# ed-fish/data-efficient-video-transformers

Measured on AMD Instinct MI355X. Metric: clips/sec fwd+bwd, B=8 T=32 3x224x224 bf16, higher is better.
Workload: dtype bf16; 1 GPU; ViViT metric shape (SURVEY 8 'M'; BASELINE configs[2]/[3] transformer): B=8/GPU, T=32, 3x224x224, patch 16, d=512, ...; global_batch=8, parallelism=dp1

## Files before the change

data-efficient-video-transformers_amd/csrc/attention.hip:

```cpp
#include "common.h"
#include <cstdlib>

namespace {

__device__ __forceinline__ void wave_lds_sync() {
  asm volatile("s_waitcnt lgkmcnt(0)" ::: "memory");
  __builtin_amdgcn_wave_barrier();
}

constexpr float kLog2e = 1.4426950408889634f;
constexpr float kLn2 = 0.6931471805599453f;

struct AttnParams {
  const void *q, *k, *v, *o, *d_o;
  void *out, *dq, *dk, *dv;
  float* lse;
  float* delta;
  int B, H, Lq, Lk, dh;
  int64_t q_sb, q_sh, q_sl, k_sb, k_sh, k_sl, v_sb, v_sh, v_sl, o_sb, o_sh, o_sl;
  float scale;
  int Lkp;
  int Lqp;
  int patch_off;
  uint32_t drop_thr;
// ... 777 lines not shown
  };
  V8 qf[2];
  load_q(wid, qf);
  stage_images<E>(ks, kb, p.k_sl, vs, vb, p.v_sl, p.Lk, NKP * 32);
  __syncthreads();

  const float c2 = p.scale * kLog2e;
  char* patch = p.patch_off >= 0 ? smem + p.patch_off + wid * 2048 : nullptr;
  for (int qt = wid; qt < nqt; qt += W) {
    asm volatile("" ::: "memory");
    f32x4 s[NKP][2];
#pragma unroll
    for (int kp = 0; kp < NKP; ++kp)
#pragma unroll
      for (int tt = 0; tt < 2; ++tt) {
        s[kp][tt] = f32x4{0.f, 0.f, 0.f, 0.f};
#pragma unroll
        for (int kk = 0; kk < 2; ++kk)
          s[kp][tt] = Elem16<E>::mma(img_row_frag<E>(ks, (2 * kp + tt) * 16, kk, g, li), qf[kk], s[kp][tt]);
      }
    load_q(qt + W, qf);
    __builtin_amdgcn_sched_barrier(0);
#pragma unroll
    for (int tt = 0; tt < 2; ++tt)
#pragma unroll
      for (int r = 0; r < 4; ++r)
        if ((2 * (NKP - 1) + tt) * 16 + 4 * g + r >= p.Lk) s[NKP - 1][tt][r] = -INFINITY;
    float mx = vmax2(s[0][0][0], s[0][0][1]);
#pragma unroll
    for (int kp = 0; kp < NKP; ++kp)
#pragma unroll
      for (int tt = 0; tt < 2; ++tt) {
        if (kp == 0 && tt == 0) {
          mx = vmax3(mx, s[0][0][2], s[0][0][3]);
        } else {
          mx = vmax3(mx, s[kp][tt][0], s[kp][tt][1]);
          mx = vmax3(mx, s[kp][tt][2], s[kp][tt][3]);
        }
      }
    mx = rows_allreduce<true>(mx);
    const float mn = mx * c2;
    f32x4 o[4];
#pragma unroll
    for (int dt = 0; dt < 4; ++dt) o[dt] = f32x4{0.f, 0.f, 0.f, 0.f};
    f32x4 ol = f32x4{0.f, 0.f, 0.f, 0.f};
    V8 ones;
#pragma unroll
    for (int j = 0; j < 8; ++j) ones[j] = (E)1.0f;
    const f32x2 c2v = {c2, c2}, mnv = {-mn, -mn};
#pragma unroll
    for (int kp = 0; kp < NKP; ++kp) {
#pragma unroll
      for (int tt = 0; tt < 2; ++tt) {
        const f32x2 a = __builtin_elementwise_fma(f32x2{s[kp][tt][0], s[kp][tt][1]}, c2v, mnv);
        const f32x2 c = __builtin_elementwise_fma(f32x2{s[kp][tt][2], s[kp][tt][3]}, c2v, mnv);
        s[kp][tt][0] = __builtin_amdgcn_exp2f(a[0]);
        s[kp][tt][1] = __builtin_amdgcn_exp2f(a[1]);
        s[kp][tt][2] = __builtin_amdgcn_exp2f(c[0]);
        s[kp][tt][3] = __builtin_amdgcn_exp2f(c[1]);
      }
      const V8 pf = pack_pair<E>(s[kp][0], s[kp][1]);
#pragma unroll
      for (int dt = 0; dt < 4; ++dt)
        o[dt] = Elem16<E>::mma(img_tr_frag<E>(vs, 2 * kp, 2 * kp + 1, dt * 16, g, li), pf, o[dt]);
      ol = Elem16<E>::mma(ones, pf, ol);
    }
    const float l = ol[0];
    const float inv = 1.0f / l;
    const int qi = qt * 16 + li;
    consume(qf[0]);
    consume(qf[1]);
    store_tile<E>(patch, ob, p.o_sl, qt * 16, p.Lq, o, inv, lane);
    if (qi < p.Lq && g == 0) lse[qi] = (mn + __builtin_amdgcn_logf(l)) * kLn2;
  }
}


template <typename E, int NKP>
__global__ __launch_bounds__(1024) void attn_bwd_dq_mfma_kernel(const AttnParams p) {
  extern __shared__ __attribute__((aligned(16))) char smem[];
  using V8 = typename Elem16<E>::v8;
  const int lane = threadIdx.x & 63, wid = threadIdx.x >> 6, W = blockDim.x >> 6;
  const int g = lane >> 4, li = lane & 15;
  const int b = blockIdx.x / p.H, h = blockIdx.x % p.H;
  const E* qb = (const E*)p.q + b * p.q_sb + h * p.q_sh;
  const E* kb = (const E*)p.k + b * p.k_sb + h * p.k_sh;
  const E* vb = (const E*)p.v + b * p.v_sb + h * p.v_sh;
  const E* ob = (const E*)p.o + b * p.o_sb + h * p.o_sh;
  const E* gb = (const E*)p.d_o + b * p.o_sb + h * p.o_sh;
  E* dqb = (E*)p.dq + b * p.q_sb + h * p.q_sh;
  const float* lse = p.lse + ((int64_t)b * p.H + h) * p.Lq;
  float* delta = p.delta + ((int64_t)b * p.H + h) * p.Lq;
  char* ks = smem;
  char* vs = smem + p.Lkp * kRowBytes;
  const int nqt = (p.Lq + 15) >> 4, nkp = NKP ? NKP : p.Lkp >> 5;
  auto load_rows = [&](int qt, V8* qf, V8* gf, V8* of, float& l2) {
    const int qi = qt * 16 + li;
    const int qrow = qi < p.Lq ? qi : p.Lq - 1;
#pragma unroll
    for (int kk = 0; kk < 2; ++kk) {
      qf[kk] = *reinterpret_cast<const V8*>(qb + (int64_t)qrow * p.q_sl + kk * 32 + g * 8);
      gf[kk] = *reinterpret_cast<const V8*>(gb + (int64_t)qrow * p.o_sl + kk * 32 + g * 8);
      of[kk] = *reinterpret_cast<const V8*>(ob + (int64_t)qrow * p.o_sl + kk * 32 + g * 8);
    }
    l2 = lse[qrow] * kLog2e;
  };
  V8 qf[2], gf[2], of[2];
  float l2;
  load_rows(wid, qf, gf, of, l2);
  stage_images<E>(ks, kb, p.k_sl, vs, vb, p.v_sl, p.Lk, p.Lkp);
  __syncthreads();

  const float c2 = p.scale * kLog2e;
  char* patch = p.patch_off >= 0 ? smem + p.patch_off + wid * 2048 : nullptr;
  for (int qt = wid; qt < nqt; qt += W) {
    asm volatile("" ::: "memory");
    float dl = 0.f;
#pragma unroll
    for (int kk = 0; kk < 2; ++kk)
#pragma unroll
      for (int j = 0; j < 8; ++j) dl = fmaf((float)gf[kk][j], (float)of[kk][j], dl);
    dl = rows_allreduce<false>(dl);
    if (g == 0 && qt * 16 + li < p.Lq) delta[qt * 16 + li] = dl;
    V8 qn[2], gn[2];
    float l2n;
    load_rows(qt + W, qn, gn, of, l2n);
    __builtin_amdgcn_sched_barrier(0);
    f32x4 acc[4];
#pragma unroll
    for (int dt = 0; dt < 4; ++dt) acc[dt] = f32x4{0.f, 0.f, 0.f, 0.f};
    const f32x2 c2v = {c2, c2}, l2v = {-l2, -l2}, dlv = {-dl, -dl};
    auto step = [&](int kp, bool last) {
      f32x4 s[2], dp[2];
#pragma unroll
      for (int tt = 0; tt < 2; ++tt) {
        s[tt] = f32x4{0.f, 0.f, 0.f, 0.f};
        dp[tt] = f32x4{0.f, 0.f, 0.f, 0.f};
#pragma unroll
        for (int kk = 0; kk < 2; ++kk) {
          s[tt] = Elem16<E>::mma(img_row_frag<E>(ks, (2 * kp + tt) * 16, kk, g, li), qf[kk], s[tt]);
          dp[tt] = Elem16<E>::mma(img_row_frag<E>(vs, (2 * kp + tt) * 16, kk, g, li), gf[kk], dp[tt]);
        }
      }
#pragma unroll
      for (int tt = 0; tt < 2; ++tt)
#pragma unroll
        for (int r = 0; r < 4; r += 2) {
          const f32x2 x = __builtin_elementwise_fma(f32x2{s[tt][r], s[tt][r + 1]}, c2v, l2v);
          const f32x2 d = f32x2{dp[tt][r], dp[tt][r + 1]} + dlv;
          const f32x2 pr = {__builtin_amdgcn_exp2f(x[0]), __builtin_amdgcn_exp2f(x[1])};
          const f32x2 ds = pr * d;
          s[tt][r] = ds[0];
          s[tt][r + 1] = ds[1];
          if (last && (2 * kp + tt) * 16 + 4 * g + r >= p.Lk) s[tt][r] = 0.f;
          if (last && (2 * kp + tt) * 16 + 4 * g + r + 1 >= p.Lk) s[tt][r + 1] = 0.f;
        }
      const V8 dsf = pack_pair<E>(s[0], s[1]);
#pragma unroll
      for (int dt = 0; dt < 4; ++dt)
        acc[dt] = Elem16<E>::mma(img_tr_frag<E>(ks, 2 * kp, 2 * kp + 1, dt * 16, g, li), dsf, acc[dt]);
    };
    if constexpr (NKP > 0) {
#pragma unroll
      for (int kp = 0; kp < NKP; ++kp) step(kp, kp == NKP - 1);
    } else {
      for (int kp = 0; kp < nkp - 1; ++kp) step(kp, false);
      step(nkp - 1, true);
    }
#pragma unroll
    for (int kk = 0; kk < 2; ++kk) {
      consume(qn[kk]);
      consume(gn[kk]);
      consume(of[kk]);
    }
    consume(l2n);
    store_tile<E>(patch, dqb, p.q_sl, qt * 16, p.Lq, acc, p.scale, lane);
#pragma unroll
    for (int kk = 0; kk < 2; ++kk) {
      qf[kk] = qn[kk];
      gf[kk] = gn[kk];
    }
    l2 = l2n;
  }
}

template <typename E, int NQP>
__global__ __launch_bounds__(1024) void attn_bwd_dkv_mfma_kernel(const AttnParams p) {
  extern __shared__ __attribute__((aligned(16))) char smem[];
  using V8 = typename Elem16<E>::v8;
  const int lane = threadIdx.x & 63, wid = threadIdx.x >> 6, W = blockDim.x >> 6;
  const int g = lane >> 4, li = lane & 15;
  const int b = blockIdx.x / p.H, h = blockIdx.x % p.H;
  const E* qb = (const E*)p.q + b * p.q_sb + h * p.q_sh;
  const E* kb = (const E*)p.k + b * p.k_sb + h * p.k_sh;
  const E* vb = (const E*)p.v + b * p.v_sb + h * p.v_sh;
  const E* gb = (const E*)p.d_o + b * p.o_sb + h * p.o_sh;
  E* dkb = (E*)p.dk + b * p.k_sb + h * p.k_sh;
  E* dvb = (E*)p.dv + b * p.v_sb + h * p.v_sh;
  const float* lse = p.lse + ((int64_t)b * p.H + h) * p.Lq;
  const float* delta = p.delta + ((int64_t)b * p.H + h) * p.Lq;
  char* qs = smem;
  char* gs = smem + p.Lqp * kRowBytes;
  float* l2s = reinterpret_cast<float*>(smem + 2 * p.Lqp * kRowBytes);
  float* dls = l2s + p.Lqp;
  const int nkt = (p.Lk + 15) >> 4, nqp = NQP ? NQP : p.Lqp >> 5;
  auto load_rows = [&](int kt, V8* kf, V8* vf) {
    const int kj = kt * 16 + li;
    const int krow = kj < p.Lk ? kj : p.Lk - 1;
#pragma unroll
    for (int kk = 0; kk < 2; ++kk) {
      kf[kk] = *reinterpret_cast<const V8*>(kb + (int64_t)krow * p.k_sl + kk * 32 + g * 8);
      vf[kk] = *reinterpret_cast<const V8*>(vb + (int64_t)krow * p.v_sl + kk * 32 + g * 8);
    }
  };
  V8 kf[2], vf[2];
  load_rows(wid, kf, vf);
  const int sr = (int)threadIdx.x < p.Lq ? (int)threadIdx.x : p.Lq - 1;
  const float lse0 = lse[sr], dl0 = delta[sr];
  stage_images<E>(qs, qb, p.q_sl, gs, gb, p.o_sl, p.Lq, p.Lqp);
  if ((int)threadIdx.x < p.Lqp) {
    l2s[threadIdx.x] = (int)threadIdx.x < p.Lq ? -lse0 * kLog2e : 0.f;
    dls[threadIdx.x] = (int)threadIdx.x < p.Lq ? -dl0 : 0.f;
  }
  for (int r = threadIdx.x + blockDim.x; r < p.Lqp; r += blockDim.x) {
    l2s[r] = r < p.Lq ? -lse[r] * kLog2e : 0.f;
    dls[r] = r < p.Lq ? -delta[r] : 0.f;
  }
  __syncthreads();

  const float c2 = p.scale * kLog2e;
  char* patch = p.patch_off >= 0 ? smem + p.patch_off + wid * 2048 : nullptr;
  for (int kt = wid; kt < nkt; kt += W) {
    asm volatile("" ::: "memory");
    f32x4 dk[4], dv[4];
#pragma unroll
    for (int dt = 0; dt < 4; ++dt) {
      dk[dt] = f32x4{0.f, 0.f, 0.f, 0.f};
      dv[dt] = f32x4{0.f, 0.f, 0.f, 0.f};
    }
    const f32x2 c2v = {c2, c2};
    auto step = [&](int qp) {
      f32x4 s[2], dp[2];
#pragma unroll
      for (int tt = 0; tt < 2; ++tt) {
        s[tt] = f32x4{0.f, 0.f, 0.f, 0.f};
        dp[tt] = f32x4{0.f, 0.f, 0.f, 0.f};
#pragma unroll
        for (int kk = 0; kk < 2; ++kk) {
          s[tt] = Elem16<E>::mma(img_row_frag<E>(qs, (2 * qp + tt) * 16, kk, g, li), kf[kk], s[tt]);
          dp[tt] = Elem16<E>::mma(img_row_frag<E>(gs, (2 * qp + tt) * 16, kk, g, li), vf[kk], dp[tt]);
        }
      }
#pragma unroll
      for (int tt = 0; tt < 2; ++tt) {
        const int q0 = (2 * qp + tt) * 16 + 4 * g;
        const f32x4 l2 = *reinterpret_cast<const f32x4*>(l2s + q0);
        const f32x4 dl = *reinterpret_cast<const f32x4*>(dls + q0);
#pragma unroll
        for (int r = 0; r < 4; r += 2) {
          const f32x2 x = __builtin_elementwise_fma(f32x2{s[tt][r], s[tt][r + 1]}, c2v, f32x2{l2[r], l2[r + 1]});
          const f32x2 d = f32x2{dp[tt][r], dp[tt][r + 1]} + f32x2{dl[r], dl[r + 1]};
          const f32x2 pr = {__builtin_amdgcn_exp2f(x[0]), __builtin_amdgcn_exp2f(x[1])};
          const f32x2 ds = pr * d;
          s[tt][r] = pr[0];
          s[tt][r + 1] = pr[1];
          dp[tt][r] = ds[0];
          dp[tt][r + 1] = ds[1];
        }
      }
      const V8 pf = pack_pair<E>(s[0], s[1]);
      const V8 dsf = pack_pair<E>(dp[0], dp[1]);
#pragma unroll
      for (int dt = 0; dt < 4; ++dt) {
        dv[dt] = Elem16<E>::mma(img_tr_frag<E>(gs, 2 * qp, 2 * qp + 1, dt * 16, g, li), pf, dv[dt]);
        dk[dt] = Elem16<E>::mma(img_tr_frag<E>(qs, 2 * qp, 2 * qp + 1, dt * 16, g, li), dsf, dk[dt]);
      }
    };
    if constexpr (NQP > 0) {
#pragma unroll
      for (int qp = 0; qp < NQP; ++qp) step(qp);
    } else {
      for (int qp = 0; qp < nqp; ++qp) step(qp);
    }
    if (kt + W < nkt) load_rows(kt + W, kf, vf);
    store_tile<E>(patch, dkb, p.k_sl, kt * 16, p.Lk, dk, p.scale, lane);
    store_tile<E>(patch, dvb, p.v_sl, kt * 16, p.Lk, dv, 1.0f, lane);
  }
}

constexpr int kStripRow = 80;

template <typename E>
__device__ __forceinline__ typename Elem16<E>::v8 strip_tr_frag(const char* strip, int ta, int tb, int col0, int g, int li) {
  const int qq = li >> 2, pp = li & 3;
  typename Elem16<E>::v4 half[2];
#pragma unroll
  for (int hf = 0; hf < 2; ++hf) {
    const int r = 16 * (hf ? tb : ta) + 4 * g + qq;
    half[hf] = Elem16<E>::tr_read(strip + r * kStripRow + col0 * 2 + 8 * pp);
  }
  return __builtin_shufflevector(half[0], half[1], 0, 1, 2, 3, 4, 5, 6, 7);
}

template <typename E, int NCH>
__device__ __forceinline__ void stage_bwd_operands(char* qs, const E* q, int64_t q_sl, char* gs, const E* g, const E* o, int64_t o_sl,
                                                   char* ks, const E* k, int64_t k_sl, int Lq, int Lk, int rows_pad, float* dls) {
  using V8 = typename Elem16<E>::v8;
  const int total = rows_pad * 8, nt = blockDim.x;
  V8 vq[NCH], vg[NCH], vo[NCH], vk[NCH];
#pragma unroll
  for (int u = 0; u < NCH; ++u) {
    const int idx = min((int)threadIdx.x + u * nt, total - 1);
    const int r = idx >> 3, c = idx & 7;
    const int rq = r < Lq ? r : 0, rk = r < Lk ? r : 0;
    vq[u] = *reinterpret_cast<const V8*>(q + (int64_t)rq * q_sl + c * 8);
    vg[u] = *reinterpret_cast<const V8*>(g + (int64_t)rq * o_sl + c * 8);
    vo[u] = *reinterpret_cast<const V8*>(o + (int64_t)rq * o_sl + c * 8);
    vk[u] = *reinterpret_cast<const V8*>(k + (int64_t)rk * k_sl + c * 8);
  }
  __builtin_amdgcn_sched_barrier(0);
  const V8 zero = {0, 0, 0, 0, 0, 0, 0, 0};
#pragma unroll
  for (int u = 0; u < NCH; ++u) {
    const int idx = min((int)threadIdx.x + u * nt, total - 1);
    const int r = idx >> 3, off = img_off(r, idx & 7);
    const bool lq = r < Lq, lk = r < Lk;
    *reinterpret_cast<V8*>(qs + off) = lq ? vq[u] : zero;
    *reinterpret_cast<V8*>(gs + off) = lq ? vg[u] : zero;
    *reinterpret_cast<V8*>(ks + off) = lk ? vk[u] : zero;
    float d = 0.f;
#pragma unroll
    for (int j = 0; j < 8; ++j) d = fmaf((float)vg[u][j], (float)vo[u][j], d);
    d += __shfl_xor(d, 1, 64);
    d += __shfl_xor(d, 2, 64);
    d += __shfl_xor(d, 4, 64);
    if ((idx & 7) == 0) dls[r] = lq ? -d : 0.f;
  }
}

template <typename E, int NP>
__global__ __launch_bounds__(512) void attn_bwd_fused_kernel(const AttnParams p) {
  extern __shared__ __attribute__((aligned(16))) char smem[];
  using V8 = typename Elem16<E>::v8;
  using V4 = typename Elem16<E>::v4;
  constexpr int LP = 32 * NP;
  const int lane = threadIdx.x & 63;
  const int wid = __builtin_amdgcn_readfirstlane(threadIdx.x >> 6);
  const int W = blockDim.x >> 6, WC = W - 1;
  const int g = lane >> 4, li = lane & 15;
  const int b = blockIdx.x / p.H, h = blockIdx.x % p.H;
  const E* qb = (const E*)p.q + b * p.q_sb + h * p.q_sh;
  const E* kb = (const E*)p.k + b * p.k_sb + h * p.k_sh;
  const E* vb = (const E*)p.v + b * p.v_sb + h * p.v_sh;
  const E* ob = (const E*)p.o + b * p.o_sb + h * p.o_sh;
  const E* gb = (const E*)p.d_o + b * p.o_sb + h * p.o_sh;
  E* dqb = (E*)p.dq + b * p.q_sb + h * p.q_sh;
  E* dkb = (E*)p.dk + b * p.k_sb + h * p.k_sh;
  E* dvb = (E*)p.dv + b * p.v_sb + h * p.v_sh;
  const float* lse = p.lse + ((int64_t)b * p.H + h) * p.Lq;
  char* qs = smem;
  char* gs = qs + LP * kRowBytes;
  char* ks = gs + LP * kRowBytes;
  char* strip0 = ks + LP * kRowBytes;
  float* l2s = reinterpret_cast<float*>(strip0 + 2 * LP * kStripRow);
  float* dls = l2s + LP;
  char* patch = reinterpret_cast<char*>(dls + LP) + wid * 2048;

  V8 kf[2][2], vf[2][2];
  if (wid < WC) {
#pragma unroll
    for (int j = 0; j < 2; ++j) {
      const int kj = (2 * wid + j) * 16 + li;
      const int krow = kj < p.Lk ? kj : p.Lk - 1;
#pragma unroll
      for (int kk = 0; kk < 2; ++kk) {
        kf[j][kk] = *reinterpret_cast<const V8*>(kb + (int64_t)krow * p.k_sl + kk * 32 + g * 8);
        vf[j][kk] = *reinterpret_cast<const V8*>(vb + (int64_t)krow * p.v_sl + kk * 32 + g * 8);
      }
    }
  }
  {
    const int r = threadIdx.x;
    const float l = lse[r < p.Lq ? r : 0];
    stage_bwd_operands<E, 4>(qs, qb, p.q_sl, gs, gb, ob, p.o_sl, ks, kb, p.k_sl, p.Lq, p.Lk, LP, dls);
    if (r < LP) l2s[r] = r < p.Lq ? -l * kLog2e : 0.f;
  }
  __syncthreads();
  const float c2 = p.scale * kLog2e;
  if (wid < WC) {
    f32x4 dk[2][4], dv[2][4];
#pragma unroll
    for (int j = 0; j < 2; ++j)
#pragma unroll
      for (int dt = 0; dt < 4; ++dt) {
        dk[j][dt] = f32x4{0.f, 0.f, 0.f, 0.f};
        dv[j][dt] = f32x4{0.f, 0.f, 0.f, 0.f};
      }
    const f32x2 c2v = {c2, c2};
    const bool kvalid[2] = {(2 * wid) * 16 + li < p.Lk, (2 * wid + 1) * 16 + li < p.Lk};
    char* myrow[2] = {strip0 + ((2 * wid) * 16 + li) * kStripRow + g * 8, strip0 + ((2 * wid + 1) * 16 + li) * kStripRow + g * 8};
#pragma unroll
    for (int qp = 0; qp < NP; ++qp) {
      asm volatile("" ::: "memory");
      V8 qfr[2][2], gfr[2][2];
#pragma unroll
      for (int tt = 0; tt < 2; ++tt)
#pragma unroll
        for (int kk = 0; kk < 2; ++kk) {
          qfr[tt][kk] = img_row_frag<E>(qs, (2 * qp + tt) * 16, kk, g, li);
          gfr[tt][kk] = img_row_frag<E>(gs, (2 * qp + tt) * 16, kk, g, li);
        }
      f32x4 l2[2], dl[2];
#pragma unroll
      for (int tt = 0; tt < 2; ++tt) {
        l2[tt] = *reinterpret_cast<const f32x4*>(l2s + (2 * qp + tt) * 16 + 4 * g);
        dl[tt] = *reinterpret_cast<const f32x4*>(dls + (2 * qp + tt) * 16 + 4 * g);
      }
      V8 pf[2], dsf[2];
#pragma unroll
      for (int j = 0; j < 2; ++j) {
        f32x4 s[2], dp[2];
#pragma unroll
        for (int tt = 0; tt < 2; ++tt) {
          s[tt] = f32x4{0.f, 0.f, 0.f, 0.f};
          dp[tt] = f32x4{0.f, 0.f, 0.f, 0.f};
#pragma unroll
          for (int kk = 0; kk < 2; ++kk) {
            s[tt] = Elem16<E>::mma(qfr[tt][kk], kf[j][kk], s[tt]);
            dp[tt] = Elem16<E>::mma(gfr[tt][kk], vf[j][kk], dp[tt]);
          }
        }
#pragma unroll
        for (int tt = 0; tt < 2; ++tt)
#pragma unroll
          for (int r = 0; r < 4; r += 2) {
            const f32x2 x = __builtin_elementwise_fma(f32x2{s[tt][r], s[tt][r + 1]}, c2v, f32x2{l2[tt][r], l2[tt][r + 1]});
            const f32x2 d = f32x2{dp[tt][r], dp[tt][r + 1]} + f32x2{dl[tt][r], dl[tt][r + 1]};
            f32x2 pr = {__builtin_amdgcn_exp2f(x[0]), __builtin_amdgcn_exp2f(x[1])};
            if (!kvalid[j]) pr = f32x2{0.f, 0.f};
            const f32x2 ds = pr * d;
            s[tt][r] = pr[0];
            s[tt][r + 1] = pr[1];
            dp[tt][r] = ds[0];
            dp[tt][r + 1] = ds[1];
          }
        pf[j] = pack_pair<E>(s[0], s[1]);
        dsf[j] = pack_pair<E>(dp[0], dp[1]);
      }
#pragma unroll
      for (int j = 0; j < 2; ++j) {
        char* row = myrow[j] + (qp & 1) * (LP * kStripRow);
        *reinterpret_cast<V4*>(row) = __builtin_shufflevector(dsf[j], dsf[j], 0, 1, 2, 3);
        *reinterpret_cast<V4*>(row + 32) = __builtin_shufflevector(dsf[j], dsf[j], 4, 5, 6, 7);
      }
#pragma unroll
      for (int dt = 0; dt < 4; ++dt) {
        const V8 gt = img_tr_frag<E>(gs, 2 * qp, 2 * qp + 1, dt * 16, g, li);
        const V8 qt = img_tr_frag<E>(qs, 2 * qp, 2 * qp + 1, dt * 16, g, li);
#pragma unroll
        for (int j = 0; j < 2; ++j) {
          dv[j][dt] = Elem16<E>::mma(gt, pf[j], dv[j][dt]);
          dk[j][dt] = Elem16<E>::mma(qt, dsf[j], dk[j][dt]);
        }
      }
      __syncthreads();
    }
#pragma unroll
    for (int j = 0; j < 2; ++j) {
      const int k0 = (2 * wid + j) * 16;
      if (k0 < p.Lk) {
        store_tile<E>(patch, dkb, p.k_sl, k0, p.Lk, dk[j], p.scale, lane);
        store_tile<E>(patch, dvb, p.v_sl, k0, p.Lk, dv[j], 1.0f, lane);
      }
    }
  } else {
    V8 ka[NP][4];
#pragma unroll
    for (int kp = 0; kp < NP; ++kp)
#pragma unroll
      for (int dt = 0; dt < 4; ++dt) ka[kp][dt] = img_tr_frag<E>(ks, 2 * kp, 2 * kp + 1, dt * 16, g, li);
#pragma unroll 1
    for (int qp = 0; qp < NP; ++qp) {
      __syncthreads();
      const char* strip = strip0 + (qp & 1) * (LP * kStripRow);
      V8 bq[NP][2];
#pragma unroll
      for (int kp = 0; kp < NP; ++kp) {
        bq[kp][0] = strip_tr_frag<E>(strip, 2 * kp, 2 * kp + 1, 0, g, li);
        bq[kp][1] = strip_tr_frag<E>(strip, 2 * kp, 2 * kp + 1, 16, g, li);
      }
      f32x4 acc[2][4];
#pragma unroll
      for (int tt = 0; tt < 2; ++tt)
#pragma unroll
        for (int dt = 0; dt < 4; ++dt) acc[tt][dt] = f32x4{0.f, 0.f, 0.f, 0.f};
#pragma unroll
      for (int kp = 0; kp < NP; ++kp)
#pragma unroll
        for (int dt = 0; dt < 4; ++dt) {
          acc[0][dt] = Elem16<E>::mma(ka[kp][dt], bq[kp][0], acc[0][dt]);
          acc[1][dt] = Elem16<E>::mma(ka[kp][dt], bq[kp][1], acc[1][dt]);
        }
#pragma unroll
      for (int tt = 0; tt < 2; ++tt)
        if ((2 * qp + tt) * 16 < p.Lq) store_tile<E>(nullptr, dqb, p.q_sl, (2 * qp + tt) * 16, p.Lq, acc[tt], p.scale, lane);
    }
  }
}

constexpr int kMaxLds = 160 * 1024;

int fill_params(const dvt_attn_desc* d, AttnParams& p, bool bwd, const char* name) {
  DVT_REQUIRE(d, "%s: null descriptor", name);
  DVT_REQUIRE(d->q && d->k && d->v && d->o && d->lse, "%s: null q/k/v/o/lse", name);
  DVT_REQUIRE(d->B >= 0 && d->H > 0 && d->Lq > 0 && d->Lk > 0 && d->dh > 0, "%s: bad sizes", name);
  DVT_REQUIRE(d->B * d->H < (1ll << 31) && d->Lq < (1 << 24) && d->Lk < (1 << 24), "%s: sizes too large", name);
  if (bwd) DVT_REQUIRE(d->d_o && d->dq && d->dk && d->dv, "%s: null gradient pointer", name);
  p.q = d->q; p.k = d->k; p.v = d->v; p.o = d->o; p.out = d->o; p.d_o = d->d_o;
  p.dq = d->dq; p.dk = d->dk; p.dv = d->dv; p.lse = d->lse; p.delta = nullptr;
  p.B = (int)d->B; p.H = (int)d->H; p.Lq = (int)d->Lq; p.Lk = (int)d->Lk; p.dh = (int)d->dh;
  p.q_sb = d->q_sb; p.q_sh = d->q_sh; p.q_sl = d->q_sl;
  p.k_sb = d->k_sb; p.k_sh = d->k_sh; p.k_sl = d->k_sl;
  p.v_sb = d->v_sb; p.v_sh = d->v_sh; p.v_sl = d->v_sl;
  p.o_sb = d->o_sb; p.o_sh = d->o_sh; p.o_sl = d->o_sl;
  p.scale = d->scale;
  DVT_REQUIRE(d->dropout_p >= 0.f && d->dropout_p < 1.f, "%s: dropout_p must be in [0, 1)", name);
  DVT_REQUIRE(d->dropout_p == 0.f || d->rng_state, "%s: dropout needs rng_state", name);
  p.drop_thr = 0u; p.drop_scale = 1.f; p.rng = d->rng_state; p.rng_off = d->rng_offset;
  if (d->dropout_p > 0.f) {
    const double th = (double)d->dropout_p * 4294967296.0;
    p.drop_thr = th >= 4294967295.0 ? 0xFFFFFFFFu : (uint32_t)(th + 0.5);
    if (p.drop_thr == 0u) p.drop_thr = 1u;
    p.drop_scale = 1.0f / (1.0f - d->dropout_p);
  }
  p.Lkp = (p.Lk + 31) & ~31;
  p.Lqp = (p.Lq + 31) & ~31;
  p.patch_off = -1;

  return DVT_OK;
}

bool strides_vec_ok(const dvt_attn_desc* d) {
  const int64_t s[] = {d->q_sb, d->q_sh, d->q_sl, d->k_sb, d->k_sh, d->k_sl,
                       d->v_sb, d->v_sh, d->v_sl, d->o_sb, d->o_sh, d->o_sl};
  for (int64_t x : s)
    if (x % 8) return false;
  return true;
}

bool mfma_fwd_ok(const dvt_attn_desc* d, const AttnParams& p) {
  return d->dropout_p == 0.f && d->scale > 0.f && dvt_is_16bit(d->dtype) && d->dh == DH && strides_vec_ok(d) && dvt_aligned16(d->q) &&
         dvt_aligned16(d->k) && dvt_aligned16(d->v) && dvt_aligned16(d->o) &&
         2 * p.Lkp * kRowBytes <= kMaxLds;
}

bool q1_ok(const dvt_attn_desc* d, const AttnParams& p) {
  return p.Lq == 1 && d->dropout_p == 0.f && dvt_is_16bit(d->dtype) && d->dh == DH && strides_vec_ok(d) &&
         dvt_aligned16(d->q) && dvt_aligned16(d->k) && dvt_aligned16(d->v) && dvt_aligned16(d->o) &&
         (size_t)4 * p.Lkp * sizeof(float) <= (size_t)kMaxLds;
}

bool mfma_bwd_ok(const dvt_attn_desc* d, const AttnParams& p) {
  return mfma_fwd_ok(d, p) && dvt_aligned16(d->d_o) && dvt_aligned16(d->dq) && dvt_aligned16(d->dk) &&
         dvt_aligned16(d->dv) && 2 * p.Lqp * kRowBytes + 2 * p.Lqp * 4 <= kMaxLds;
}

bool fused_bwd_ok(const AttnParams& p) { return p.Lqp == p.Lkp && p.Lkp <= 224; }
size_t fused_bwd_lds(int NP, int waves) {
  const size_t LP = 32 * (size_t)NP;
  return 3 * LP * kRowBytes + 2 * LP * kStripRow + 2 * LP * sizeof(float) + (size_t)waves * 2048;
}

int pick_waves(int tiles, size_t lds_bytes, int cap = 16) {
  int maxw = lds_bytes > 80 * 1024 ? 16 : 8;
  if (maxw > cap) maxw = cap;
  const int rounds = (tiles + maxw - 1) / maxw;
  int w = (tiles + rounds - 1) / rounds;
  return w < 1 ? 1 : w;
}

size_t with_patches(size_t lds, int waves, AttnParams& p) {
  const size_t tot = lds + (size_t)waves * 2048;
  const bool ok = lds <= 80 * 1024 ? 2 * tot <= (size_t)kMaxLds : tot <= (size_t)kMaxLds;
  p.patch_off = ok ? (int)lds : -1;
  return ok ? tot : lds;
}

template <typename K>
int set_lds(K kernel, size_t bytes) {
  if (bytes > 64 * 1024) {
    const hipError_t e = hipFuncSetAttribute((const void*)kernel, hipFuncAttributeMaxDynamicSharedMemorySize, (int)bytes);
    if (e != hipSuccess) return dvt_fail_hip(e, "hipFuncSetAttribute(MaxDynamicSharedMemorySize)");
  }
  return 0;
}

int resolve_fwd(const dvt_attn_desc* d, AttnParams& p, dvt_attn_plan_info& r) {
  r = dvt_attn_plan_info{};
  r.patch = r.patch2 = -1;
  int rc = fill_params(d, p, false, "dvt_attention_fwd");
  if (rc) return rc;
  if (p.B == 0) return DVT_OK;
  if (q1_ok(d, p)) {
    r.family = DVT_ATTN_F_Q1; r.waves = 4; r.lds = (int64_t)4 * p.Lkp * sizeof(float);
    return DVT_OK;
  }
  if (mfma_fwd_ok(d, p)) {
    const size_t lds_img = (size_t)2 * p.Lkp * kRowBytes;
    const int nkp = p.Lkp >> 5;
    r.waves = pick_waves((p.Lq + 15) / 16, lds_img, nkp > 7 && nkp <= 11 ? 12 : 16);
    r.lds = (int64_t)with_patches(lds_img, r.waves, p);
    r.patch = p.patch_off >= 0;
    r.family = nkp <= 11 ? DVT_ATTN_F_RES : DVT_ATTN_F_ONLINE;
    r.count = nkp <= 11 ? nkp : 0;
    return DVT_OK;
  }
  const int nt_s = p.Lq * p.dh >= 4096 ? 512 : 256;
  const size_t lds_s = ((size_t)(p.Lq + 2 * p.Lk) * small_dhp(p.dh) +
                        (size_t)small_parts(p.Lq, p.Lk, nt_s) * p.Lq * small_lp(p.Lk)) * sizeof(float);
  if (d->dtype != DVT_F32 && d->dtype != DVT_BF16 && d->dtype != DVT_F16)
    DVT_UNSUPPORTED("dvt_attention_fwd: dtype %d not supported", d->dtype);
  if (p.Lq <= kSmallL && p.Lk <= kSmallL && p.dh <= kSmallDh && lds_s <= (size_t)kMaxLds) {
    r.family = DVT_ATTN_F_SMALL; r.waves = nt_s / 64; r.lds = (int64_t)lds_s;
    return DVT_OK;
  }
  const size_t lds = (size_t)4 * (p.dh + p.Lk) * sizeof(float);
  if (lds > (size_t)kMaxLds) DVT_UNSUPPORTED("dvt_attention_fwd: Lk = %d, dh = %d exceed the LDS budget", p.Lk, p.dh);
  r.family = DVT_ATTN_F_GENERIC; r.waves = 4; r.lds = (int64_t)lds;
  return DVT_OK;
}

int resolve_bwd(const dvt_attn_desc* d, AttnParams& p, AttnParams& pq, AttnParams& pkv, dvt_attn_plan_info& r) {
  r = dvt_attn_plan_info{};
  r.patch = r.patch2 = -1;
  int rc = fill_params(d, p, true, "dvt_attention_bwd");
  if (rc) return rc;
  pq = pkv = p;
  if (p.B == 0) return DVT_OK;
  if (q1_ok(d, p) && dvt_aligned16(d->d_o) && dvt_aligned16(d->dq) && dvt_aligned16(d->dk) && dvt_aligned16(d->dv)) {
    r.family = DVT_ATTN_B_Q1; r.waves = 4;
    return DVT_OK;
  }
  if (mfma_bwd_ok(d, p) && fused_bwd_ok(p) && !d->bwd_two_pass) {
    const int NP = p.Lkp >> 5;
    r.family = DVT_ATTN_B_FUSED; r.count = NP;
    r.waves = NP + 1;
    r.lds = (int64_t)fused_bwd_lds(NP, r.waves);
    return DVT_OK;
  }
  if (mfma_bwd_ok(d, p)) {
    const size_t img_q = (size_t)2 * p.Lkp * kRowBytes;
    const size_t img_kv = (size_t)2 * p.Lqp * kRowBytes + (size_t)2 * p.Lqp * sizeof(float);
    r.family = DVT_ATTN_B_PAIR; r.workspace = 1;
    r.count = (p.Lkp >> 5) <= 11 ? p.Lkp >> 5 : 0;
    r.count2 = (p.Lqp >> 5) <= 11 ? p.Lqp >> 5 : 0;
    r.waves = pick_waves((p.Lq + 15) / 16, img_q);
    r.waves2 = pick_waves((p.Lk + 15) / 16, img_kv);
    r.lds = (int64_t)with_patches(img_q, r.waves, pq);
    r.lds2 = (int64_t)with_patches(img_kv, r.waves2, pkv);
    r.patch = pq.patch_off >= 0; r.patch2 = pkv.patch_off >= 0;
    return DVT_OK;
  }
  if (d->dtype != DVT_F32 && d->dtype != DVT_BF16 && d->dtype != DVT_F16)
    DVT_UNSUPPORTED("dvt_attention_bwd: dtype %d not supported", d->dtype);
  const int nt_s = p.Lq * p.dh >= 4096 ? 512 : 256;
  const size_t lds_s = ((size_t)2 * (p.Lq + p.Lk) * small_dhp(p.dh) +
                        (size_t)2 * small_parts(p.Lq, p.Lk, nt_s) * p.Lq * small_lp(p.Lk) +
                        (size_t)2 * p.Lk * small_lp(p.Lq)) * sizeof(float);
  if (p.Lq <= kSmallL && p.Lk <= kSmallL && p.dh <= kSmallDh && lds_s <= (size_t)kMaxLds) {
    r.family = DVT_ATTN_B_SMALL; r.waves = nt_s / 64; r.lds = (int64_t)lds_s;
    return DVT_OK;
  }
  const size_t lds_q = (size_t)4 * (2 * p.dh + p.Lk) * sizeof(float);
  const size_t lds_kv = (size_t)4 * (2 * p.dh + 2 * p.Lq) * sizeof(float);
  if (lds_q > (size_t)kMaxLds || lds_kv > (size_t)kMaxLds)
    DVT_UNSUPPORTED("dvt_attention_bwd: Lq = %d, Lk = %d, dh = %d exceed the LDS budget", p.Lq, p.Lk, p.dh);
  r.family = DVT_ATTN_B_GENERIC; r.workspace = 1; r.waves = r.waves2 = 4;
  r.lds = (int64_t)lds_q; r.lds2 = (int64_t)lds_kv;
  return DVT_OK;
}

}

extern "C" {

size_t dvt_attention_bwd_workspace_bytes(const dvt_attn_desc* d) {
  if (!d) return 0;
  return (size_t)d->B * (size_t)d->H * (size_t)d->Lq * sizeof(float);
}

int dvt_attention_plan(const dvt_attn_desc* d, int bwd, dvt_attn_plan_info* info) {
  DVT_REQUIRE(info, "dvt_attention_plan: null info");
  AttnParams p, pq, pkv;
  return bwd ? resolve_bwd(d, p, pq, pkv, *info) : resolve_fwd(d, p, *info);
}

int dvt_attention_fwd(const dvt_attn_desc* d, dvt_stream_t stream) {
  AttnParams p;
  dvt_attn_plan_info r;
  int rc = resolve_fwd(d, p, r);
  if (rc) return rc;
  if (p.B == 0) return DVT_OK;
  hipStream_t st = (hipStream_t)stream;
  const size_t lds = (size_t)r.lds;
  if (r.family == DVT_ATTN_F_Q1) {
    const dim3 grid((unsigned)dvt_cdiv((int64_t)p.B * p.H, 4)), block(256);
    DVT_DISPATCH_16BIT(d->dtype, E, {
      if (int rc_ = set_lds(attn_fwd_q1_kernel<E>, lds)) return rc_;
      hipLaunchKernelGGL((attn_fwd_q1_kernel<E>), grid, block, lds, st, p);
    });
    DVT_LAUNCH_CHECK("dvt_attention_fwd(q1)");
    return DVT_OK;
  }
  if (r.family == DVT_ATTN_F_RES || r.family == DVT_ATTN_F_ONLINE) {
    const dim3 grid((unsigned)(p.B * p.H)), block(64 * r.waves);
#define DVT_ATTN_FWD_RES(NKP)                                                               \
  case NKP:                                                                                 \
    if (int rc_ = set_lds(attn_fwd_mfma_res_kernel<E, NKP>, lds)) return rc_;                                         \
    hipLaunchKernelGGL((attn_fwd_mfma_res_kernel<E, NKP>), grid, block, lds, st, p);        \
    break
    DVT_DISPATCH_16BIT(d->dtype, E, {
      switch (r.count) {
        DVT_ATTN_FWD_RES(1); DVT_ATTN_FWD_RES(2); DVT_ATTN_FWD_RES(3); DVT_ATTN_FWD_RES(4);
        DVT_ATTN_FWD_RES(5); DVT_ATTN_FWD_RES(6); DVT_ATTN_FWD_RES(7); DVT_ATTN_FWD_RES(8);
        DVT_ATTN_FWD_RES(9); DVT_ATTN_FWD_RES(10); DVT_ATTN_FWD_RES(11);
        default:
          if (int rc_ = set_lds(attn_fwd_mfma_kernel<E>, lds)) return rc_;
          hipLaunchKernelGGL((attn_fwd_mfma_kernel<E>), grid, block, lds, st, p);
      }
    });
#undef DVT_ATTN_FWD_RES
    DVT_LAUNCH_CHECK("dvt_attention_fwd(mfma)");
    return DVT_OK;
  }
  if (r.family == DVT_ATTN_F_SMALL) {
    const dim3 grid((unsigned)(p.B * p.H)), block(64 * r.waves);
#define DVT_ATTN_SMALL_FWD(T)                                                   \
  do {                                                                          \
    if (int rc_ = set_lds(attn_small_fwd_kernel<T>, lds)) return rc_;                                   \
    hipLaunchKernelGGL((attn_small_fwd_kernel<T>), grid, block, lds, st, p);  \
  } while (0)
    if (d->dtype == DVT_F32) DVT_ATTN_SMALL_FWD(float);
    else if (d->dtype == DVT_BF16) DVT_ATTN_SMALL_FWD(bf16);
    else DVT_ATTN_SMALL_FWD(f16);
#undef DVT_ATTN_SMALL_FWD
    DVT_LAUNCH_CHECK("dvt_attention_fwd(short)");
    return DVT_OK;
  }
  const int64_t rows = (int64_t)p.B * p.H * p.Lq;
  const dim3 grid((unsigned)dvt_cdiv(rows, 4)), block(256);
  if (d->dtype == DVT_F32) {
    if (int rc_ = set_lds(attn_fwd_generic_kernel<float>, lds)) return rc_;
    hipLaunchKernelGGL((attn_fwd_generic_kernel<float>), grid, block, lds, st, p);
  } else if (d->dtype == DVT_BF16) {
    if (int rc_ = set_lds(attn_fwd_generic_kernel<bf16>, lds)) return rc_;
    hipLaunchKernelGGL((attn_fwd_generic_kernel<bf16>), grid, block, lds, st, p);
  } else {
    if (int rc_ = set_lds(attn_fwd_generic_kernel<f16>, lds)) return rc_;
    hipLaunchKernelGGL((attn_fwd_generic_kernel<f16>), grid, block, lds, st, p);
  }
  DVT_LAUNCH_CHECK("dvt_attention_fwd(generic)");
  return DVT_OK;
}

int dvt_attention_bwd(const dvt_attn_desc* d, dvt_stream_t stream) {
  AttnParams p, pq, pkv;
  dvt_attn_plan_info r;
  int rc = resolve_bwd(d, p, pq, pkv, r);
  if (rc) return rc;
  if (p.B == 0) return DVT_OK;
  hipStream_t st = (hipStream_t)stream;
  if (r.family == DVT_ATTN_B_Q1) {
    const dim3 grid((unsigned)dvt_cdiv((int64_t)p.B * p.H, 4)), block(256);
    DVT_DISPATCH_16BIT(d->dtype, E, hipLaunchKernelGGL((attn_bwd_q1_kernel<E>), grid, block, 0, st, p));
    DVT_LAUNCH_CHECK("dvt_attention_bwd(q1)");
    return DVT_OK;
  }
  if (r.family == DVT_ATTN_B_FUSED) {
    const size_t lds = (size_t)r.lds;
    const dim3 grid((unsigned)(p.B * p.H)), block(64 * r.waves);
#define DVT_ATTN_BWD_FUSED(N)                                                               \
  case N:                                                                                   \
    if (int rc_ = set_lds(attn_bwd_fused_kernel<E, N>, lds)) return rc_;                                              \
    hipLaunchKernelGGL((attn_bwd_fused_kernel<E, N>), grid, block, lds, st, p);             \
    break
    DVT_DISPATCH_16BIT(d->dtype, E, {
      switch (r.count) {
        DVT_ATTN_BWD_FUSED(1); DVT_ATTN_BWD_FUSED(2); DVT_ATTN_BWD_FUSED(3); DVT_ATTN_BWD_FUSED(4);
        DVT_ATTN_BWD_FUSED(5); DVT_ATTN_BWD_FUSED(6); DVT_ATTN_BWD_FUSED(7);
      }
    });
#undef DVT_ATTN_BWD_FUSED
    DVT_LAUNCH_CHECK("dvt_attention_bwd(fused)");
    return DVT_OK;
  }
  if (r.family == DVT_ATTN_B_PAIR) {
    DVT_REQUIRE(d->workspace, "dvt_attention_bwd: workspace (dvt_attention_bwd_workspace_bytes) required");
    pq.delta = pkv.delta = (float*)d->workspace;
    const dim3 grid((unsigned)(p.B * p.H));
    const dim3 block_q(64 * r.waves), block_kv(64 * r.waves2);
    const size_t lds_q = (size_t)r.lds, lds_kv = (size_t)r.lds2;
#define DVT_ATTN_BWD_DQ(NKP)                                                                \
  case NKP:                                                                                 \
    if (int rc_ = set_lds(attn_bwd_dq_mfma_kernel<E, NKP>, lds_q)) return rc_;                                        \
    hipLaunchKernelGGL((attn_bwd_dq_mfma_kernel<E, NKP>), grid, block_q, lds_q, st, pq);     \
    break
#define DVT_ATTN_BWD_DKV(NQP)                                                               \
  case NQP:                                                                                 \
    if (int rc_ = set_lds(attn_bwd_dkv_mfma_kernel<E, NQP>, lds_kv)) return rc_;                                      \
    hipLaunchKernelGGL((attn_bwd_dkv_mfma_kernel<E, NQP>), grid, block_kv, lds_kv, st, pkv);  \
    break
    DVT_DISPATCH_16BIT(d->dtype, E, {
      switch (r.count) {
        DVT_ATTN_BWD_DQ(1); DVT_ATTN_BWD_DQ(2); DVT_ATTN_BWD_DQ(3); DVT_ATTN_BWD_DQ(4);
        DVT_ATTN_BWD_DQ(5); DVT_ATTN_BWD_DQ(6); DVT_ATTN_BWD_DQ(7); DVT_ATTN_BWD_DQ(8);
        DVT_ATTN_BWD_DQ(9); DVT_ATTN_BWD_DQ(10); DVT_ATTN_BWD_DQ(11);
        default:
          if (int rc_ = set_lds(attn_bwd_dq_mfma_kernel<E, 0>, lds_q)) return rc_;
          hipLaunchKernelGGL((attn_bwd_dq_mfma_kernel<E, 0>), grid, block_q, lds_q, st, pq);
      }
      switch (r.count2) {
        DVT_ATTN_BWD_DKV(1); DVT_ATTN_BWD_DKV(2); DVT_ATTN_BWD_DKV(3); DVT_ATTN_BWD_DKV(4);
        DVT_ATTN_BWD_DKV(5); DVT_ATTN_BWD_DKV(6); DVT_ATTN_BWD_DKV(7); DVT_ATTN_BWD_DKV(8);
        DVT_ATTN_BWD_DKV(9); DVT_ATTN_BWD_DKV(10); DVT_ATTN_BWD_DKV(11);
        default:
          if (int rc_ = set_lds(attn_bwd_dkv_mfma_kernel<E, 0>, lds_kv)) return rc_;
          hipLaunchKernelGGL((attn_bwd_dkv_mfma_kernel<E, 0>), grid, block_kv, lds_kv, st, pkv);
      }
    });
#undef DVT_ATTN_BWD_DQ
#undef DVT_ATTN_BWD_DKV
    DVT_LAUNCH_CHECK("dvt_attention_bwd(dkdv)");
    return DVT_OK;
  }
  if (r.family == DVT_ATTN_B_SMALL) {
    const size_t lds_s = (size_t)r.lds;
    const dim3 grid((unsigned)(p.B * p.H)), block(64 * r.waves);
#define DVT_ATTN_SMALL_BWD(T)                                                   \
  do {                                                                          \
    if (int rc_ = set_lds(attn_small_bwd_kernel<T>, lds_s)) return rc_;                                   \
    hipLaunchKernelGGL((attn_small_bwd_kernel<T>), grid, block, lds_s, st, p);  \
  } while (0)
    if (d->dtype == DVT_F32) DVT_ATTN_SMALL_BWD(float);
    else if (d->dtype == DVT_BF16) DVT_ATTN_SMALL_BWD(bf16);
    else DVT_ATTN_SMALL_BWD(f16);
#undef DVT_ATTN_SMALL_BWD
    DVT_LAUNCH_CHECK("dvt_attention_bwd(short)");
    return DVT_OK;
  }
  DVT_REQUIRE(d->workspace, "dvt_attention_bwd: workspace (dvt_attention_bwd_workspace_bytes) required");
  p.delta = (float*)d->workspace;
  const size_t lds_q = (size_t)r.lds, lds_kv = (size_t)r.lds2;
  const int64_t qrows = (int64_t)p.B * p.H * p.Lq, krows = (int64_t)p.B * p.H * p.Lk;
  const dim3 block(256);
#define DVT_ATTN_BWD_GENERIC(T)                                                                   \
  do {                                                                                            \
    if (int rc_ = set_lds(attn_bwd_dq_generic_kernel<T>, lds_q)) return rc_;                                                \
    if (int rc_ = set_lds(attn_bwd_dkv_generic_kernel<T>, lds_kv)) return rc_;                                              \
    hipLaunchKernelGGL((attn_delta_kernel<T>), dim3((unsigned)dvt_cdiv(qrows, 4)), block, 0, st, p); \
    hipLaunchKernelGGL((attn_bwd_dq_generic_kernel<T>), dim3((unsigned)dvt_cdiv(qrows, 4)), block, lds_q, st, p); \
    hipLaunchKernelGGL((attn_bwd_dkv_generic_kernel<T>), dim3((unsigned)dvt_cdiv(krows, 4)), block, lds_kv, st, p); \
  } while (0)
  if (d->dtype == DVT_F32) DVT_ATTN_BWD_GENERIC(float);
  else if (d->dtype == DVT_BF16) DVT_ATTN_BWD_GENERIC(bf16);
  else DVT_ATTN_BWD_GENERIC(f16);
#undef DVT_ATTN_BWD_GENERIC
  DVT_LAUNCH_CHECK("dvt_attention_bwd(generic)");
  return DVT_OK;
}

}
```

Baseline: 1414 clips/s.

## Stream Q/dO/O strips into LDS via async DMA pipelined with fused attention backward

```diff
diff --git a/data-efficient-video-transformers_amd/csrc/attention.hip b/data-efficient-video-transformers_amd/csrc/attention.hip
--- a/data-efficient-video-transformers_amd/csrc/attention.hip
+++ b/data-efficient-video-transformers_amd/csrc/attention.hip
@@ -1103,39 +1103,59 @@
   return __builtin_shufflevector(half[0], half[1], 0, 1, 2, 3, 4, 5, 6, 7);
 }
 
-template <typename E, int NCH>
-__device__ __forceinline__ void stage_bwd_operands(char* qs, const E* q, int64_t q_sl, char* gs, const E* g, const E* o, int64_t o_sl,
-                                                   char* ks, const E* k, int64_t k_sl, int Lq, int Lk, int rows_pad, float* dls) {
+#pragma clang diagnostic push
+#pragma clang diagnostic ignored "-Winline-asm"
+typedef int bwd_raw16 __attribute__((ext_vector_type(4)));
+__device__ __forceinline__ void load16_uncounted(bwd_raw16& dst, const void* src) {
+  asm volatile("global_load_dwordx4 %0, %1, off" : "=v"(dst) : "v"(src) : "memory");
+}
+__device__ __forceinline__ void load4_uncounted(float& dst, const void* src) {
+  asm volatile("global_load_dword %0, %1, off" : "=v"(dst) : "v"(src) : "memory");
+}
+#pragma clang diagnostic pop
+
+template <int STEP, int MAXK, int K = 0>
+__device__ __forceinline__ void wait_vm_multiple(int k) {
+  static_assert(STEP * MAXK < 64, "vmcnt is a 6-bit counter");
+  if constexpr (K == MAXK) dvt_wait_vm<STEP * MAXK>();
+  else if (k == K) dvt_wait_vm<STEP * K>();
+  else wait_vm_multiple<STEP, MAXK, K + 1>(k);
+}
+
+__device__ __forceinline__ int img_chunk_of_slot(int r, int slot) { return (((slot >> 1) ^ ((r >> 1) & 3)) << 1) | (slot & 1); }
+
+template <typename E, int NP>
+__device__ __forceinline__ void stage_bwd_operands(int s, int slot, int lane, char* qs, const E* q, int64_t q_sl, char* gs, const E* g,
+                                                   char* os, const E* o, int64_t o_sl, int Lq) {
+  for (int j = slot; j < 4; j += NP) {
+    const int r0 = 32 * s + 8 * j, r = r0 + (lane >> 3), rq = r < Lq ? r : 0;
+    const int c = img_chunk_of_slot(r, lane & 7);
+    dvt_dma16(q + (int64_t)rq * q_sl + c * 8, qs + r0 * kRowBytes);
+    dvt_dma16(g + (int64_t)rq * o_sl + c * 8, gs + r0 * kRowBytes);
+    dvt_dma16(o + (int64_t)rq * o_sl + (lane & 7) * 8, os + r0 * kRowBytes);
+  }
+}
+
+template <typename E, int NP>
+__device__ __forceinline__ void finish_bwd_strip(int s, int slot, int lane, char* qs, char* gs, const char* os, float* dls, int Lq) {
   using V8 = typename Elem16<E>::v8;
-  const int total = rows_pad * 8, nt = blockDim.x;
-  V8 vq[NCH], vg[NCH], vo[NCH], vk[NCH];
-#pragma unroll
-  for (int u = 0; u < NCH; ++u) {
-    const int idx = min((int)threadIdx.x + u * nt, total - 1);
-    const int r = idx >> 3, c = idx & 7;
-    const int rq = r < Lq ? r : 0, rk = r < Lk ? r : 0;
-    vq[u] = *reinterpret_cast<const V8*>(q + (int64_t)rq * q_sl + c * 8);
-    vg[u] = *reinterpret_cast<const V8*>(g + (int64_t)rq * o_sl + c * 8);
-    vo[u] = *reinterpret_cast<const V8*>(o + (int64_t)rq * o_sl + c * 8);
-    vk[u] = *reinterpret_cast<const V8*>(k + (int64_t)rk * k_sl + c * 8);
-  }
-  __builtin_amdgcn_sched_barrier(0);
-  const V8 zero = {0, 0, 0, 0, 0, 0, 0, 0};
-#pragma unroll
-  for (int u = 0; u < NCH; ++u) {
-    const int idx = min((int)threadIdx.x + u * nt, total - 1);
-    const int r = idx >> 3, off = img_off(r, idx & 7);
-    const bool lq = r < Lq, lk = r < Lk;
-    *reinterpret_cast<V8*>(qs + off) = lq ? vq[u] : zero;
-    *reinterpret_cast<V8*>(gs + off) = lq ? vg[u] : zero;
-    *reinterpret_cast<V8*>(ks + off) = lk ? vk[u] : zero;
+  for (int j = slot; j < 4; j += NP) {
+    const int r0 = 32 * s + 8 * j, r = r0 + (lane >> 3), c = lane & 7;
+    const V8 vg = *reinterpret_cast<const V8*>(gs + img_off(r, c));
+    const V8 vo = *reinterpret_cast<const V8*>(os + r0 * kRowBytes + lane * 16);
     float d = 0.f;
 #pragma unroll
-    for (int j = 0; j < 8; ++j) d = fmaf((float)vg[u][j], (float)vo[u][j], d);
+    for (int e = 0; e < 8; ++e) d = fmaf((float)vg[e], (float)vo[e], d);
     d += __shfl_xor(d, 1, 64);
     d += __shfl_xor(d, 2, 64);
     d += __shfl_xor(d, 4, 64);
-    if ((idx & 7) == 0) dls[r] = lq ? -d : 0.f;
+    if (c == 0) dls[r] = r < Lq ? -d : 0.f;
+    if (r0 + 8 > Lq) {
+      if (r >= Lq) {
+        *reinterpret_cast<V8*>(qs + r0 * kRowBytes + lane * 16) = V8{0, 0, 0, 0, 0, 0, 0, 0};
+        *reinterpret_cast<V8*>(gs + r0 * kRowBytes + lane * 16) = V8{0, 0, 0, 0, 0, 0, 0, 0};
+      }
+    }
   }
 }
 
@@ -1145,9 +1165,13 @@
   using V8 = typename Elem16<E>::v8;
   using V4 = typename Elem16<E>::v4;
   constexpr int LP = 32 * NP;
+  constexpr int WC = NP;
+  constexpr int kStripDma = 3 * (NP >= 4 ? 1 : 4 / NP);
+  constexpr int kKDma = 4;
+  constexpr int kDepth = NP > 1 ? 1 : 0;
   const int lane = threadIdx.x & 63;
   const int wid = __builtin_amdgcn_readfirstlane(threadIdx.x >> 6);
-  const int W = blockDim.x >> 6, WC = W - 1;
+  const int slot = NP >= 5 ? (wid < NP - 4 ? wid : wid == NP - 4 ? 4 : wid - 1) : wid;
   const int g = lane >> 4, li = lane & 15;
   const int b = blockIdx.x / p.H, h = blockIdx.x % p.H;
   const E* qb = (const E*)p.q + b * p.q_sb + h * p.q_sh;
@@ -1165,30 +1189,50 @@
   char* strip0 = ks + LP * kRowBytes;
   float* l2s = reinterpret_cast<float*>(strip0 + 2 * LP * kStripRow);
   float* dls = l2s + LP;
-  char* patch = reinterpret_cast<char*>(dls + LP) + wid * 2048;
-
-  V8 kf[2][2], vf[2][2];
+  char* os = reinterpret_cast<char*>(dls + LP);
+  char* patch = os + wid * 2048;
+
+  const float c2 = p.scale * kLog2e;
   if (wid < WC) {
+    bwd_raw16 kraw[2][2], vraw[2][2];
+    float lraw;
 #pragma unroll
     for (int j = 0; j < 2; ++j) {
       const int kj = (2 * wid + j) * 16 + li;
       const int krow = kj < p.Lk ? kj : p.Lk - 1;
 #pragma unroll
       for (int kk = 0; kk < 2; ++kk) {
-        kf[j][kk] = *reinterpret_cast<const V8*>(kb + (int64_t)krow * p.k_sl + kk * 32 + g * 8);
-        vf[j][kk] = *reinterpret_cast<const V8*>(vb + (int64_t)krow * p.v_sl + kk * 32 + g * 8);
-      }
-    }
-  }
-  {
-    const int r = threadIdx.x;
-    const float l = lse[r < p.Lq ? r : 0];
-    stage_bwd_operands<E, 4>(qs, qb, p.q_sl, gs, gb, ob, p.o_sl, ks, kb, p.k_sl, p.Lq, p.Lk, LP, dls);
-    if (r < LP) l2s[r] = r < p.Lq ? -l * kLog2e : 0.f;
-  }
-  __syncthreads();
-  const float c2 = p.scale * kLog2e;
-  if (wid < WC) {
+        load16_uncounted(kraw[j][kk], kb + (int64_t)krow * p.k_sl + kk * 32 + g * 8);
+        load16_uncounted(vraw[j][kk], vb + (int64_t)krow * p.v_sl + kk * 32 + g * 8);
+      }
+    }
+    const int tr = threadIdx.x;
+    load4_uncounted(lraw, lse + (tr < p.Lq ? tr : 0));
+    stage_bwd_operands<E, NP>(0, slot, lane, qs, qb, p.q_sl, gs, gb, os, ob, p.o_sl, p.Lq);
+    auto request_k = [&]() {
+#pragma unroll
+      for (int t = 0; t < kKDma; ++t) {
+        const int r0 = 32 * wid + 8 * t, r = r0 + (lane >> 3), rk = r < p.Lk ? r : 0;
+        dvt_dma16(kb + (int64_t)rk * p.k_sl + img_chunk_of_slot(r, lane & 7) * 8, ks + r0 * kRowBytes);
+      }
+    };
+    dvt_wait_vm<0>();
+    asm volatile("" : "+v"(kraw[0][0]), "+v"(kraw[0][1]), "+v"(kraw[1][0]), "+v"(kraw[1][1]), "+v"(vraw[0][0]),
+                      "+v"(vraw[0][1]), "+v"(vraw[1][0]), "+v"(vraw[1][1]), "+v"(lraw));
+    V8 kf[2][2], vf[2][2];
+#pragma unroll
+    for (int j = 0; j < 2; ++j)
+#pragma unroll
+      for (int kk = 0; kk < 2; ++kk) {
+        kf[j][kk] = __builtin_bit_cast(V8, kraw[j][kk]);
+        vf[j][kk] = __builtin_bit_cast(V8, vraw[j][kk]);
+      }
+    finish_bwd_strip<E, NP>(0, slot, lane, qs, gs, os, dls, p.Lq);
+    if (tr < LP) l2s[tr] = tr < p.Lq ? -lraw * kLog2e : 0.f;
+    __syncthreads();
+    request_k();
+#pragma unroll
+    for (int s = 1; s <= kDepth; ++s) stage_bwd_operands<E, NP>(s, slot, lane, qs, qb, p.q_sl, gs, gb, os, ob, p.o_sl, p.Lq);
     f32x4 dk[2][4], dv[2][4];
 #pragma unroll
     for (int j = 0; j < 2; ++j)
@@ -1203,6 +1247,8 @@
 #pragma unroll
     for (int qp = 0; qp < NP; ++qp) {
       asm volatile("" ::: "memory");
+      if (qp + kDepth + 1 < NP)
+        stage_bwd_operands<E, NP>(qp + kDepth + 1, slot, lane, qs, qb, p.q_sl, gs, gb, os, ob, p.o_sl, p.Lq);
       V8 qfr[2][2], gfr[2][2];
 #pragma unroll
       for (int tt = 0; tt < 2; ++tt)
@@ -1264,6 +1310,20 @@
           dk[j][dt] = Elem16<E>::mma(qt, dsf[j], dk[j][dt]);
         }
       }
+      if (qp + 1 < NP) {
+        if (slot < 4) wait_vm_multiple<kStripDma, kDepth>(NP - 2 - qp);
+        else dvt_wait_vm<0>();
+        finish_bwd_strip<E, NP>(qp + 1, slot, lane, qs, gs, os, dls, p.Lq);
+      } else if (NP == 1) {
+        dvt_wait_vm<0>();
+      }
+      if (qp == 0 && 32 * wid + 32 > p.Lk) {
+#pragma unroll
+        for (int t = 0; t < kKDma; ++t) {
+          const int r0 = 32 * wid + 8 * t;
+          if (r0 + (lane >> 3) >= p.Lk) *reinterpret_cast<V8*>(ks + r0 * kRowBytes + lane * 16) = V8{0, 0, 0, 0, 0, 0, 0, 0};
+        }
+      }
       __syncthreads();
     }
 #pragma unroll
@@ -1275,6 +1335,8 @@
       }
     }
   } else {
+    __syncthreads();
+    __syncthreads();
     V8 ka[NP][4];
 #pragma unroll
     for (int kp = 0; kp < NP; ++kp)
@@ -1282,7 +1344,7 @@
       for (int dt = 0; dt < 4; ++dt) ka[kp][dt] = img_tr_frag<E>(ks, 2 * kp, 2 * kp + 1, dt * 16, g, li);
 #pragma unroll 1
     for (int qp = 0; qp < NP; ++qp) {
-      __syncthreads();
+      if (qp) __syncthreads();
       const char* strip = strip0 + (qp & 1) * (LP * kStripRow);
       V8 bq[NP][2];
 #pragma unroll
@@ -1369,7 +1431,8 @@
 bool fused_bwd_ok(const AttnParams& p) { return p.Lqp == p.Lkp && p.Lkp <= 224; }
 size_t fused_bwd_lds(int NP, int waves) {
   const size_t LP = 32 * (size_t)NP;
-  return 3 * LP * kRowBytes + 2 * LP * kStripRow + 2 * LP * sizeof(float) + (size_t)waves * 2048;
+  const size_t tail = LP * kRowBytes > (size_t)waves * 2048 ? LP * kRowBytes : (size_t)waves * 2048;
+  return 3 * LP * kRowBytes + 2 * LP * kStripRow + 2 * LP * sizeof(float) + tail;
 }
 
 int pick_waves(int tiles, size_t lds_bytes, int cap = 16) {
```

Result: no change. 1412 clips/s (-0.1%).
